# EndlessReform/fish-speech.rs

Measured on AMD Instinct MI355X. Metric: codec tokens/sec (frames/s; 1 frame = 1 slow + 8 codebook tokens = 2048 PCM samples), Fish-1.5 batch=1, higher is better.
Workload: dtype bf16

## Files before the change

fish-speech.rs_amd/csrc/lm_engine.hip:

```cpp
#include "lm_engine.h"

#include <algorithm>
#include <array>
#include <cmath>
#include <cstdlib>
#include <cstring>
#include <chrono>
#include <condition_variable>
#include <initializer_list>
#include <map>
#include <mutex>
#include <type_traits>
#include <vector>

#include <fcntl.h>
#include <sys/file.h>
#include <sys/stat.h>
#include <unistd.h>

#include "fs_common.h"
#include "fs_synth.h"
#include "lm_kernels.h"
#include "lm_persist.h"
#include "lm_persist_rows.h"
// ... 135 lines not shown
            throw Error("no HIP device visible: libfishrt has no CPU fallback (MI355X / gfx950 required)");
        FS_REQUIRE(device >= 0 && device < ndev, "device_id out of range");
        FS_HIP(hipSetDevice(device));
        hipDeviceProp_t prop;
        FS_HIP(hipGetDeviceProperties(&prop, device));
        if (std::string(prop.gcnArchName).rfind("gfx950", 0) != 0)
            throw Error(std::string("libfishrt kernels are built for gfx950 only; device reports ") + prop.gcnArchName);
        FS_HIP(hipStreamCreateWithFlags(&st_, hipStreamNonBlocking));
        d_.dim = a.dim; d_.inter = a.intermediate_size; d_.H = a.n_head; d_.Hk = a.n_local_heads; d_.Dh = a.head_dim;
        d_.n_rep = a.n_head / a.n_local_heads; d_.eps = a.norm_eps;
        legacy_ = !t.has_semantic_end;
        generic_ = !legacy_ && t.im_end_id + 1 != t.semantic_start_id;
        if (!legacy_) FS_REQUIRE(t.semantic_start_id >= 1 && t.semantic_start_id < (uint32_t)a.vocab_size, "semantic_start_id outside the vocabulary");
        n_audio_ = legacy_ ? 2 : (generic_ ? a.vocab_size - (int)t.semantic_start_id + 1 : a.vocab_size - (int)t.im_end_id);
        if (legacy_) FS_REQUIRE(t.pad_id < (uint32_t)a.vocab_size, "pad_id outside the vocabulary");
        plan_tensors();
        alloc_runtime();
        for (auto& e : ev_) FS_HIP(hipEventCreate(&e));
        for (auto& e : ev_batch_) FS_HIP(hipEventCreateWithFlags(&e, hipEventDisableTiming));
    }
    ~LM() override {
        (void)hipSetDevice(device_);
        (void)hipStreamSynchronize(st_);
        destroy_graphs();
        for (auto& e : ev_) if (e) (void)hipEventDestroy(e);
        for (auto& e : ev_batch_) if (e) (void)hipEventDestroy(e);
        if (h_pin_) (void)hipHostFree(h_pin_);
        for (auto& hb : hid_pool_) (void)hipFree(hb.first);
        for (const HidSlot& h : sess_hid_) if (h.rows) (void)hipFree(h.rows);
        for (auto* q : {&sess_flight_, &sess_queue_})
// ... 313 lines not shown
            use_persist_ = plock.owns_lock() && persist_ok_ && batch_rows_ == 0 &&
                           (cfg.temp == 0.f || fast_persist_samples(cfg.temp, cfg.top_k, a_.codebook_size));
            use_pslow_ = plock.owns_lock() && pslow_ok_;
        }
        if (hidden_out && !d_hidden_.p) d_hidden_.alloc(sizeof(float) * (size_t)out_cap_ * a_.dim);
        float* hid_dev = hidden_out ? d_hidden_.as<float>() : nullptr;
        FS_HIP(hipMemcpyAsync(d_hid_slot_.p, &hid_dev, sizeof(hid_dev), hipMemcpyHostToDevice, st_));
        RngState rng;
        upload_rng(seed, rng, d_rng_.as<RngState>(), st_);
        SeqState ss = {};
        ss.pos = n_cached; ss.prompt_L = L;
        FS_HIP(hipMemcpyAsync(state(0), &ss, sizeof(ss), hipMemcpyHostToDevice, st_));
        FS_HIP(hipMemcpyAsync(d_prompt_.p, prompt, sizeof(uint32_t) * C1 * L, hipMemcpyHostToDevice, st_));
        launch_reppen_reset(rp_, C, a_.codebook_size, st_);
        clear_fast();

        stats_ = {};
        FS_HIP(hipEventRecord(ev_[0], st_));
        prefill_tokens(0, L - 1, true);
        LmKernels<WT>::embed(d_, tok_emb_, cb_emb_, C, a_.codebook_size, d_cfg_.as<SampleCfg>(), d_prompt_.as<uint32_t>(), state(0),
                             x(0), st_);
        GenRun g;
        g.T0 = n_cached + L; g.n_iter = n_iter; g.cb = cb; g.cb_user = cb_user;
        g.time_k = (flags & FS_GEN_TIME_KERNELS) && use_persist_ && use_pslow_ && fold_slow_sampler();
        if constexpr (std::is_same<WT, bf16_t>::value) {
            if (getenv("FISHRT_B1_ROWS_FAST") && use_persist_ && use_pslow_ && fold_slow_sampler() && !legacy_) {
                ensure_rows(2);
                g.b1_rows_fast = true;
                const int big = 1 << 30;
                FS_HIP(hipMemcpyAsync(d_rcfg_.p, &cfg, sizeof(cfg), hipMemcpyHostToDevice, st_));
// ... 54 lines not shown

    struct GenRun {
        int T0 = 0;
        long long n_iter = 0;
        fs_frame_cb cb = nullptr;
        void* cb_user = nullptr;
        bool time_k = false, b1_rows_fast = false, multi_ok = false;
        std::vector<hipEvent_t> kev;
        long long it = 1;
        size_t delivered = 0;
        bool stop = false, ended = false;
    };
    void gen_frame(GenRun& g, long long it_) {
        set_bucket(g.T0 + (int)it_);
        if (g.b1_rows_fast) {
            launch_slow_persist(pslow_args(), st_);
            RowsFastArgs F = rows_fast_args(0, 1);
            F.slow_logits = d_logits_slow_.as<float>();
            F.cap = nullptr;
            launch_rows_fast(F, 1, persist_sampled_, st_);
            return;
        }
        if (g.time_k && it_ >= 1) {
            for (int i = 0; i < 3; ++i) { hipEvent_t e; FS_HIP(hipEventCreate(&e)); g.kev.push_back(e); }
            FS_HIP(hipEventRecord(g.kev[g.kev.size() - 3], st_));
            launch_slow_persist(pslow_args(), st_);
            FS_HIP(hipEventRecord(g.kev[g.kev.size() - 2], st_));
            launch_fast_persist(persist_args(), persist_sampled_, st_);
            FS_HIP(hipEventRecord(g.kev[g.kev.size() - 1], st_));
            return;
        }
// ... 1606 lines not shown
                if (FP8) d_sscl_.alloc(sizeof(float) * slow_persist_scale_floats(a_.n_layer));
                d_snorms_.alloc(sizeof(float) * (size_t)(2 * a_.n_layer + 1) * a_.dim);
                d_sedges_.alloc(slow_persist_edge_bytes());
                FS_HIP(hipMemset(d_sedges_.p, 0, d_sedges_.n));
                d_sctl_.alloc(320);
                FS_HIP(hipMemset(d_sctl_.p, 0, d_sctl_.n));
            }
            std::vector<const float*> np;
            for (int l = 0; l < a_.n_layer; ++l) { np.push_back(slow_[l].attn_norm); np.push_back(slow_[l].ffn_norm); }
            np.push_back(norm_w_);
            if (FP8) launch_slow_persist_pack_fp8(slow_.data(), a_.n_layer, slow_head_w(), slow_head_s(), n_audio_, np.data(), d_spack_.p, d_hpack_.p,
                                                  d_sscl_.as<float>(), d_snorms_.as<float>(), st_);
            else launch_slow_persist_pack(slow_.data(), a_.n_layer, slow_head_w(), n_audio_, np.data(), d_spack_.p, d_hpack_.p, d_snorms_.as<float>(), st_);
            FS_HIP(hipStreamSynchronize(st_));
            pslow_ok_ = true;
        }
    }
    SlowPersistArgs pslow_args() {
        SlowPersistArgs A = {};
        A.wpack = d_spack_.p; A.hpack = d_hpack_.p; A.norms = d_snorms_.as<float>();
        A.scales = d_sscl_.p ? d_sscl_.as<float>() : nullptr;
        A.hscales = d_sscl_.p ? d_sscl_.as<float>() + (size_t)a_.n_layer * PF_BLOCKS * 48 : nullptr;
        A.n_layer = a_.n_layer; A.n_head_rows = n_audio_;
        A.cos_t = d_cos_.as<float>(); A.sin_t = d_sin_.as<float>(); A.eps = d_.eps;
        A.x = x(0); A.logits = d_logits_slow_.as<float>(); A.state = state(0);
        A.kv_pool = kv_pool_.p; A.layer_half = (size_t)n_pages_ * page_elems_;
        A.page_table = d_page_table_.as<int>();
        A.n_sl = std::min(nc_launch_, nc_launch_ > 32 ? 16 : 8);
        if (const char* c = getenv("FISHRT_NSL_MAX")) A.n_sl = std::max(1, std::min(A.n_sl, atoi(c)));
        if (const char* c = getenv("FISHRT_NSL_MIN")) A.n_sl = std::min(16, std::max(A.n_sl, atoi(c)));
        while (A.n_sl & (A.n_sl - 1)) A.n_sl &= A.n_sl - 1;
        A.edges = d_sedges_.as<unsigned long long>();
        A.ctl = d_sctl_.as<uint32_t>();
        A.prof = getenv("FISHRT_PERSIST_PROF") ? reinterpret_cast<unsigned long long*>(d_sctl_.as<uint32_t>() + 16) : nullptr;
        A.peer_stamps = (A.prof && d_ctl_.p) ? reinterpret_cast<const unsigned long long*>(d_ctl_.as<uint32_t>() + 16) + 16 : nullptr;
        set_naps(A.naps, "FISHRT_NAPS_SLOW", kFp8 ? kNapsSlowFp8 : kNapsSlow);
        A.prof_wg = getenv("FISHRT_PERSIST_PROF_WG") ? atoi(getenv("FISHRT_PERSIST_PROF_WG")) : 0;
        A.l2_touch = getenv("FISHRT_SLOW_EARLY") ? atoi(getenv("FISHRT_SLOW_EARLY")) : (kFp8 ? 1 : 9);
        return A;
    }
    bool fold_slow_sampler() const { return use_persist_ && n_audio_ <= 2048; }
    FastPersistArgs persist_args() {
        FastPersistArgs A = {};
        A.wpack = d_pack_.p;
        A.scales = d_fscl_.p ? d_fscl_.as<float>() : nullptr;
        for (int l = 0; l < PF_LAYERS; ++l) { A.norms[2 * l] = fast_[l].attn_norm; A.norms[2 * l + 1] = fast_[l].ffn_norm; }
        A.norms[2 * PF_LAYERS] = fast_norm_w_;
        A.fast_emb = fast_emb_; A.tok_emb = tok_emb_; A.cb_emb = cb_emb_;
        A.qkv0_tbl = d_qkv0_.p ? d_qkv0_.as<float>() : nullptr;
        A.cos_t = d_cos_.as<float>(); A.sin_t = d_sin_.as<float>();
        A.eps = d_.eps;
        const bool fold = fold_slow_sampler();
        A.xf = fold ? x(0) : xf(0); A.x = x(0);
        A.slow_logits = fold ? d_logits_slow_.as<float>() : nullptr; A.n_slow = n_audio_; A.hid_slot = d_hid_slot_.as<float*>();
        A.cap = d_cap_.as<float>(); A.cap_frames = cap_frames_;
        A.state = state(0); A.cfg = d_cfg_.as<SampleCfg>(); A.rp = rp_; A.rng = d_rng_.as<RngState>();
        A.out_codes = d_out_.as<uint32_t>(); A.out_cap = out_cap_;
        A.edges = d_edges_.as<unsigned long long>();
        A.ctl = d_ctl_.as<uint32_t>();
        A.prof = getenv("FISHRT_PERSIST_PROF") ? reinterpret_cast<unsigned long long*>(d_ctl_.as<uint32_t>() + 16) : nullptr;
        A.peer_stamps = (A.prof && d_sctl_.p) ? reinterpret_cast<const unsigned long long*>(d_sctl_.as<uint32_t>() + 16) + 16 : nullptr;
        set_naps(A.naps, "FISHRT_NAPS_FAST", persist_sampled_ ? kNapsFastSampled : kNapsFast);
        return A;
    }


    void ensure_rows(int R) {
        if constexpr (std::is_same<WT, bf16_t>::value || kFp8) {
// ... 75 lines not shown
        A.slow_logits = d_rlogits_.as<float>() + (size_t)r0 * PR_LD; A.n_slow = n_audio_;
        A.cap = cap_frames_ ? d_rcap_.as<float>() + (size_t)r0 * cap_frames_ * 9 * 2048 : nullptr; A.cap_frames = cap_frames_;
        A.state = state(r0); A.cfg = d_rcfg_.as<SampleCfg>() + r0; A.budget = d_rbudget_.as<int>() + r0; A.rng = d_rrng_.as<RngState>() + r0;
        const RepPenState rp = rows_rp(r0);
        A.rp_mask = rp.mask; A.rp_ring = rp.ring; A.rp_meta = rp.ring_meta;
        A.out_codes = d_out_.as<uint32_t>() + (size_t)r0 * a_.num_codebooks * out_cap_; A.out_cap = out_cap_;
        A.edges = d_redges_f_.as<unsigned long long>();
        A.ctl = d_rctl_f_.as<uint32_t>();
        A.prof = getenv("FISHRT_PERSIST_PROF") ? reinterpret_cast<unsigned long long*>(d_rctl_f_.as<uint32_t>() + 16) : nullptr;
        set_naps(A.naps, "FISHRT_NAPS_ROWS_FAST", kNapsRowsFast);
        A.nap_draw = getenv("FISHRT_NAP_ROWS_DRAW") ? atoi(getenv("FISHRT_NAP_ROWS_DRAW")) : 16;
        return A;
    }
    FastPersistArgs persist_args(int i) {
        FastPersistArgs A = persist_args();
        A.xf = x(i); A.x = x(i);
        A.slow_logits = d_rlogits_.as<float>() + (size_t)i * PR_LD;
        A.cap = cap_frames_ ? d_rcap_.as<float>() + (size_t)i * cap_frames_ * 9 * 2048 : nullptr;
        A.state = state(i); A.cfg = d_rcfg_.as<SampleCfg>() + i; A.rp = rows_rp(i); A.rng = d_rrng_.as<RngState>() + i;
        A.out_codes = d_out_.as<uint32_t>() + (size_t)i * a_.num_codebooks * out_cap_;
        return A;
    }

    void enqueue_slow_layers(int b) {
        for (int l = 0; l < a_.n_layer; ++l) {
            const LayerW& w = slow_[l];
            KVView kv = slow_kv(l, b);
            LmKernels<WT>::qkv(d_, x(b), w, d_cos_.as<float>(), d_sin_.as<float>(), state(b), 0, 0, d_q_.as<float>(), kv, st_);
            LmKernels<WT>::attn_decode(d_, d_q_.as<float>(), kv, state(b), d_part_.as<float>(), n_chunks_, nc_launch_, st_);
            LmKernels<WT>::wo(d_, d_part_.as<float>(), n_chunks_, nc_launch_, state(b), nullptr, kv, 0, w, x(b), st_);
            LmKernels<WT>::ffn_up(d_, x(b), w, d_act_.as<float>(), st_);
// ... 102 lines not shown
            launch_fast_persist(persist_args(), persist_sampled_, st_);
        }
        FS_HIP(hipStreamEndCapture(st_, &g));
        FS_HIP(hipGraphInstantiate(&ge, g, nullptr, nullptr, 0));
        FS_HIP(hipGraphDestroy(g));
        multi_graphs_[key] = ge;
        return ge;
    }
    size_t page_elems_ = 0;
    DevBuf kv_pool_, fast_pool_, d_page_table_, d_zero_table_;
    std::vector<int> free_pages_, seq_len_, fast_len_;
    std::vector<std::vector<int>> seq_pages_;
    DevBuf d_x_, d_xf_, d_q_, d_part_, d_act_, d_logits_slow_, d_logits_fast_, d_state_, d_cfg_, d_rng_, d_prompt_, d_out_;
    DevBuf d_rp_mask_, d_rp_seen_, d_rp_ring_, d_rp_meta_;
    DevBuf d_pack_, d_edges_, d_ctl_, d_qkv0_;
    DevBuf d_fscl_, d_sscl_;
    DevBuf d_cap_;
    int cap_frames_ = 0;
    DevBuf d_hidden_, d_hid_slot_;
    bool persist_ok_ = false, use_persist_ = false, pslow_ok_ = false, use_pslow_ = false, persist_sampled_ = false;
    int batch_rows_ = 0, batch_row_ = 0;
    bool sess_active_ = false, sess_rows_ = false, sess_sampled_ = false;
    bool sess_slots_ = false;
    SampleCfg sess_cfg_ = {};
    DevBuf d_scfg_, d_srng_, d_srp_mask_, d_srp_seen_, d_srp_ring_, d_srp_meta_;
    int sess_R_ = 0, sess_adds_ = 0, sess_budget_tmp_ = 0;
    uint64_t sess_seed_ = 0;
    std::unique_lock<PersistLock> sess_plock_;
    std::vector<int> sess_left_, sess_pos_;
    std::vector<SeqState> sess_hs_;
// ... 72 lines not shown
```

fish-speech.rs_amd/csrc/lm_persist.h:

```cpp
#pragma once
#include <hip/hip_runtime.h>

#include <cstdint>

#include "lm_kernels.h"

namespace fs {

constexpr int PF_BLOCKS = 256;
constexpr int PF_THREADS = 512;
constexpr int PF_REPL = 8;
constexpr int PF_EDGE_CAP = 4096;
constexpr int PF_RING = 4;
constexpr int PF_LAYERS = 4;
constexpr int PF_REG_DW = PF_LAYERS * (5 + 4 + 32) + 4;
constexpr int PF_REG_CHUNKS = PF_REG_DW / 4;
constexpr int PF_ROW_CHUNKS = (PF_LAYERS * 9 + 4) / 4;
constexpr int PF_LDS_CHUNKS = PF_LAYERS * 4;
constexpr int PF_CHUNKS = PF_REG_CHUNKS + PF_LDS_CHUNKS;
constexpr int PF_SCL = 200;

struct FastPersistArgs {
    const void* wpack;
    const float* scales;
    const float* norms[2 * PF_LAYERS + 1];
    const void* fast_emb;
    const float* qkv0_tbl;
    const void* tok_emb;
    const void* cb_emb;
    const float* cos_t;
    const float* sin_t;
    float eps;
    const float* xf;
    const float* slow_logits;
    int n_slow;
    float* cap;
    int cap_frames;
    float* const* hid_slot;
    float* x;
    SeqState* state;
    const SampleCfg* cfg;
    RepPenState rp;
    RngState* rng;
    uint32_t* out_codes;
    int out_cap;
    unsigned long long* edges;
    unsigned long long* prof;
    const unsigned long long* peer_stamps;
    uint32_t* ctl;
    int naps[6];
};

constexpr int PS_EDGE_CAP = 16 * 16 * 66 + 64;
constexpr size_t PS_LAYER_IMAGE = 116736;
// ... 12 lines not shown
    const float* sin_t;
    float eps;
    float* x;
    float* logits;
    const SeqState* state;
    void* kv_pool;
    size_t layer_half;
    const int* page_table;
    int n_sl;
    unsigned long long* edges;
    unsigned long long* prof;
    const unsigned long long* peer_stamps;
    uint32_t* ctl;
    int naps[6];
    int prof_wg;
    int l2_touch;
};
size_t slow_persist_pack_bytes(int n_layer, bool fp8 = false);
size_t slow_persist_scale_floats(int n_layer);
void launch_slow_persist_pack_fp8(const LayerW* layers, int n_layer, const void* head_w, const float* head_s, int n_head_rows,
                                  const float* const* norm_ptrs, void* wpack, void* hpack, float* scales, float* norms_flat, hipStream_t st);
size_t slow_persist_edge_bytes();
void launch_slow_persist_pack(const LayerW* layers, int n_layer, const void* head_w, int n_head_rows, const float* const* norm_ptrs,
                              void* wpack, void* hpack, float* norms_flat, hipStream_t st);
void launch_slow_persist(const SlowPersistArgs& a, hipStream_t st);

bool fast_persist_supported(const ModelDims& d, int n_fast_layer, int n_cb, int cb_size);
size_t fast_persist_pack_bytes();
size_t fast_persist_edge_bytes();
void launch_fast_persist_pack(const LayerW* fast, const void* head_w, void* pack, hipStream_t st, bool fp8 = false, const float* head_s = nullptr,
// ... 10 lines not shown
```

fish-speech.rs_amd/csrc/lm_persist.hip:

```cpp
#include "lm_persist.h"

#include <hip/hip_runtime.h>

#include "fs_common.h"

namespace fs {

namespace {

#include "lm_persist_dev.h"
#include "lm_bsample_dev.h"

typedef __bf16 bf16x8_t __attribute__((ext_vector_type(8)));
typedef float f32x4_t __attribute__((ext_vector_type(4)));

constexpr int L_W2 = 0;
constexpr int L_KC = L_W2 + PF_LDS_CHUNKS * PF_THREADS * 16;
constexpr int L_VC = L_KC + PF_LAYERS * 8 * 64 * 4;
constexpr int L_QS = L_VC + PF_LAYERS * 8 * 64 * 4;
constexpr int L_XS = L_QS + 4096;
constexpr int PF_RED = 40;
constexpr int L_RED = L_XS + 4096;
constexpr int L_SC = L_RED + 2 * 8 * PF_RED * 4;
constexpr int L_AMAX = L_SC + 16 * 8 * 4;
// ... 223 lines not shown
            __syncthreads();
        }
        if (cap && tid == 0) cap[2047] = (float)idx;
        cur0 = audio_tok(cfg, max(idx, 0));
        if (cur0 == cfg.im_end_id) done_in = 1;
    }
    const bool eos = cur0 == cfg.im_end_id;
    if (eos && b != 0) return;

    bool dead = false;
    float x0 = 0.f, x1 = 0.f;
    unsigned long long tk[16] = {0, 0, 0, 0, 0, 0, 0, 0, 0, 0, 0, 0, 0, 0, 0, 0}, t_last = A.prof ? wall_clock64() : 0;
    const unsigned long long t_timers = t_last;
#define PF_TICK(k) do { if (A.prof) { const unsigned long long n_ = wall_clock64(); tk[k] += n_ - t_last; t_last = n_; } } while (0)
    if (!eos) {
        const u32x4* wp = reinterpret_cast<const u32x4*>(A.wpack) + (size_t)b * PF_CHUNKS * PF_THREADS + tid;
        uint32_t wr[4 * PF_ROW_CHUNKS];
        u32x4 w13v[PF_LAYERS][8];
#pragma unroll
        for (int c = 0; c < PF_ROW_CHUNKS; ++c) {
            const u32x4 t4 = wp[(size_t)c * PF_THREADS];
            wr[4 * c] = t4.x; wr[4 * c + 1] = t4.y; wr[4 * c + 2] = t4.z; wr[4 * c + 3] = t4.w;
        }
#pragma unroll
        for (int c = PF_ROW_CHUNKS; c < PF_REG_CHUNKS; ++c) w13v[(c - PF_ROW_CHUNKS) / 8][(c - PF_ROW_CHUNKS) % 8] = wp[(size_t)c * PF_THREADS];
#pragma unroll
        for (int c = 0; c < PF_LDS_CHUNKS; ++c) w2s[c * PF_THREADS + tid] = wp[(size_t)(PF_REG_CHUNKS + c) * PF_THREADS];
        float2 nwr[2 * PF_LAYERS + 1];
        if (!SAMPLED) {
#pragma unroll
// ... 11 lines not shown
            const float2 xin = *reinterpret_cast<const float2*>(A.xf + 2 * tid);
            x0 = xin.x; x1 = xin.y;
        }
        asm volatile("s_waitcnt vmcnt(0)" ::: "memory");
#pragma unroll
        for (int d = 0; d < 4 * PF_ROW_CHUNKS; ++d) asm volatile("" : "+v"(wr[d]));
#pragma unroll
        for (int l = 0; l < PF_LAYERS; ++l)
#pragma unroll
            for (int u2 = 0; u2 < 8; ++u2) asm volatile("" : "+v"(w13v[l][u2]));

        PF_TICK(0);
        unsigned e = 0;
        const unsigned tag0 = epoch * 256u;
        int par = 0;
        float2 tq = make_float2(0.f, 0.f), tk2 = tq, tv2 = tq;
        float xres_tbl = 0.f;
#pragma unroll 1
        for (int cb = 0; cb < 8; ++cb) {
            const int T = cb + 1;
#pragma unroll
            for (int l = 0; l < PF_LAYERS; ++l) {
                const uint32_t* wl = wr + 9 * l;
                const bool from_tbl = l == 0 && cb > 0 && A.qkv0_tbl != nullptr;
                if (!from_tbl) {
                    tid = pf_opaque(tid_k); lane = tid & 63; wave = tid >> 6;
                    const float2 nw = norm_w(2 * l, tid);
                    if (l > 0) {
                        u32x4 v;
                        pf_nap_before_sweep(A.naps[0]);
                        pf_sweep1(my_edges + (size_t)(e & 3) * PF_REPL * PF_EDGE_CAP, tid, tag0 + e + 1, v, dead, A.ctl);
                        x0 = __uint_as_float(v.x); x1 = __uint_as_float(v.z);
                        ++e;
                        PF_TICK(9);
                    }
                    if ((unsigned)(2 * tid - 4 * b) < 4u) *reinterpret_cast<float2*>(xr + 2 * tid - 4 * b) = make_float2(x0, x1);
                    const float xn0 = x0 * nw.x, xn1 = x1 * nw.y;
                    float a8[8];
#pragma unroll
// ... 313 lines not shown
                        tk2 = *reinterpret_cast<const float2*>(row + 1024 + g2 * 64 + 2 * j2);
                        tv2 = *reinterpret_cast<const float2*>(row + 1152 + g2 * 64 + 2 * j2);
                        const uint32_t hw = reinterpret_cast<const uint16_t*>(A.fast_emb)[(size_t)code * 1024 + 4 * b + min(tid & 15, 3)];
                        xres_tbl = __uint_as_float(hw << 16);
                    } else {
                        const uint32_t ew = reinterpret_cast<const uint32_t*>(A.fast_emb)[(size_t)code * 512 + tid];
                        x0 = bf_lo(ew); x1 = bf_hi(ew);
                    }
                }
            }
        }
    } else if (tid < 8) {
        s_misc[4 + tid] = 0;
        A.state->cur[tid + 1] = 0;
    }
    if (b != 0) return;
    __syncthreads();
    uint32_t* cur = s_prev;
    if (tid == 0) cur[0] = cur0;
    else if (tid <= 8) cur[tid] = s_misc[3 + tid];
    __syncthreads();
    if (tid == 0) {
        SeqState* st = A.state;
        const int frame = st->frame;
        if (done_in == 1) st->done = 2;
        if (A.slow_logits) st->cur[0] = cur0;
        if (frame == 0 || cur0 != cfg.im_end_id) {
            const int o = st->n_out;
            if (o < A.out_cap)
                for (int cc = 0; cc < 8; ++cc) A.out_codes[(size_t)cc * A.out_cap + o] = cur[cc + 1];
            st->n_out = o + 1;
        }
        for (int i = 0; i <= 8; ++i) st->prev[i] = cur[i];
        st->have_prev = 1;
        st->pos += 1;
        st->frame = frame + 1;
        if (SAMPLED || (cfg.legacy && A.slow_logits)) A.rng->consumed = consumed0 + (unsigned long long)n_draws;
        A.ctl[0] = epoch + 1;
    }
    {
        const uint32_t sem = cur[0];
        const float m = (sem >= cfg.sem_lo && sem <= cfg.sem_hi) ? 1.f : 0.f;
        const uint32_t* te = reinterpret_cast<const uint32_t*>(A.tok_emb);
        const uint32_t* ce = reinterpret_cast<const uint32_t*>(A.cb_emb);
        const uint32_t w0 = te[(size_t)sem * 512 + tid];
        float e0 = 0.f + bf_lo(w0), e1 = 0.f + bf_hi(w0);
#pragma unroll
        for (int c = 0; c < 8; ++c) {
            const uint32_t wv = ce[((size_t)c * 1024 + cur[c + 1]) * 512 + tid];
            e0 += bf_lo(wv) * m;
            e1 += bf_hi(wv) * m;
        }
        *reinterpret_cast<float2*>(A.x + 2 * tid) = make_float2(e0, e1);
    }
    PF_TICK(7);
    if (A.prof && tid == 0) {
        for (int k = 0; k < 16; ++k) A.prof[k] += tk[k];
        const unsigned long long t_end = wall_clock64(), peer_end = A.peer_stamps ? A.peer_stamps[0] : 0;
        if (peer_end && t_entry > peer_end && t_entry - peer_end < 20000) { A.prof[17] += t_entry - peer_end; A.prof[20] += 1; }
        A.prof[18] += t_timers - t_entry;
        A.prof[19] += t_end - t_last;
        A.prof[16] = t_end;
    }
#undef PF_TICK
}

__global__ __launch_bounds__(64) void k_pf_reduce_selftest(const float* __restrict__ in, float* __restrict__ out) {
    const int lane = threadIdx.x;
    float v32[32], v16[16], v8[8], v4[4];
// ... 63 lines not shown
```

fish-speech.rs_amd/csrc/lm_persist_slow.hip:

```cpp
#include "lm_persist.h"

#include <hip/hip_runtime.h>

#include <type_traits>
#include <vector>

#include "fs_common.h"

namespace fs {

namespace {

#include "lm_persist_dev.h"
#include "lm_persist_rows_dev.h"

constexpr int PS_DROR8 = 0x128;

constexpr size_t IM_QKV4 = 0, IM_QKV1 = 8192, IM_WO = 10240, IM_W13 = 18432, IM_W2 = 83968;
static_assert(IM_W2 + 4 * 8192 == PS_LAYER_IMAGE, "image layout");
constexpr size_t I8_QKV4 = 0, I8_QKV1 = 4096, I8_WO = 6144, I8_W13 = 10240, I8_W2 = 43008;
static_assert(I8_W2 + 2 * 8192 == PS_LAYER_IMAGE_FP8, "fp8 image layout");
constexpr int PS_SC = 48, SC_QKV = 0, SC_WO = 8, SC_W13 = 12, SC_W2 = 44;

typedef float f32x2_t __attribute__((ext_vector_type(2)));
// ... 165 lines not shown
    const unsigned epoch = A.ctl[0];
    const unsigned tag0 = epoch * 256u;
    const int n_sl = A.n_sl;
    const bool att = b < 16 * n_sl;
    const int ah = att ? b / n_sl : 0, as = att ? b % n_sl : 0, ag = ah >> 3;
    const int chunk_t = (pos + n_sl - 1) / n_sl;
    const int t0 = min(pos, as * chunk_t), t1 = min(pos, (as + 1) * chunk_t);
    const bool last_slice = att && as == n_sl - 1;
    const int n_tok = t1 - t0;
    const int n_tiles = att ? max((n_tok + 127) / 128, last_slice ? 1 : 0) : 0;
    if (att) {
        const int p0 = t0 >> 6;
        for (int i = tid; i < 160; i += PF_THREADS) s_pages[i] = (n_tok > 0 && p0 + i <= ((t1 - 1) >> 6)) ? A.page_table[p0 + i] : 0;
    }
    const int page_new = A.page_table[pos >> 6];
    float2 x2 = *reinterpret_cast<const float2*>(A.x + 2 * tid);
    float x0 = x2.x, x1 = x2.y;
    float rope_c = A.cos_t[(size_t)rpos * 32 + (tid & 31)], rope_s = A.sin_t[(size_t)rpos * 32 + (tid & 31)];
    __syncthreads();
    asm volatile("" : "+v"(rope_c), "+v"(rope_s));

    constexpr size_t LIMG = FP8 ? PS_LAYER_IMAGE_FP8 : PS_LAYER_IMAGE;
    const unsigned char* wimg = reinterpret_cast<const unsigned char*>(A.wpack) + (size_t)b * LIMG;
    const size_t layer_img = (size_t)PF_BLOCKS * LIMG;
    u32x4 wq4 = u32x4{0, 0, 0, 0}, wo4 = u32x4{0, 0, 0, 0}, w13[8], w2r[4];
    u32x2 wq4f = u32x2{0, 0}, wo4f = u32x2{0, 0};
    u32x4 w13f[4], w2f[2];
    uint32_t wq1;
    if constexpr (FP8) {
        wq4f = reinterpret_cast<const u32x2*>(wimg + I8_QKV4)[tid];
        wq1 = reinterpret_cast<const uint32_t*>(wimg + I8_QKV1)[tid];
    } else {
        wq4 = reinterpret_cast<const u32x4*>(wimg + IM_QKV4)[tid];
        wq1 = reinterpret_cast<const uint32_t*>(wimg + IM_QKV1)[tid];
    }
// ... 65 lines not shown
        const unsigned char* wl = wimg + (size_t)l * layer_img;
        {
            tid = pf_opaque(tid_k); lane = tid & 63; wave = tid >> 6;
            const float2 nw = *reinterpret_cast<const float2*>(A.norms + (size_t)(2 * l) * 1024 + 2 * tid);
            if (l > 0) {
                u32x4 v;
                pf_nap_before_sweep(A.naps[0]);
                pf_sweep1(my_edges + (size_t)(e & 3) * ering, tid, tag0 + e + 1, v, dead, A.ctl);
                x0 = __uint_as_float(v.x); x1 = __uint_as_float(v.z);
                ++e;
                PS_TICK(9);
            }
            const bool kv_late = (early_mode & 8) != 0;
            if (att && n_tok > 0 && !kv_late) load_kv_tile0(l);
            *reinterpret_cast<float2*>(xs + 2 * tid) = make_float2(x0, x1);
            const float xn0 = x0 * nw.x, xn1 = x1 * nw.y;
            float a8[8] = {0.f, 0.f, 0.f, 0.f, 0.f, 0.f, 0.f, 0.f};
            float rsc = 1.f;
            if constexpr (FP8) {
                if (tid < 64) rsc = scl[(size_t)l * scl_layer + SC_QKV + min(tid & 15, 4)];
                pf_dot2x2_fp8(wq4f.x, xn0, xn1, a8[0], a8[1]); pf_dot2x2_fp8(wq4f.y, xn0, xn1, a8[2], a8[3]);
                pf_dot2x2_fp8(wq1, xn0, xn1, a8[4], a8[6]);
                a8[6] = 0.f;
            } else {
                a8[0] = pf_dot2(wq4.x, xn0, xn1, 0.f); a8[1] = pf_dot2(wq4.y, xn0, xn1, 0.f);
                a8[2] = pf_dot2(wq4.z, xn0, xn1, 0.f); a8[3] = pf_dot2(wq4.w, xn0, xn1, 0.f);
                a8[4] = pf_dot2(wq1, xn0, xn1, 0.f);
            }
            a8[5] = fmaf(x1, x1, fmaf(x0, x0, 0.f));
            const float r8 = pf_reduce<8>(a8, lane);
            if ((lane & 7) == 0) red[(par * 8 + wave) * PS_RED + (lane >> 3)] = r8;
            __syncthreads();
            if (wave == 0) {
                const int r = min(lane & 15, 5), k = lane >> 4;
                const float* rp = red + (par * 8 + k) * PS_RED;
                float t = pf_sum_rows(rp[r] + rp[4 * PS_RED + r]);
                const float tot = pf_sum_rows(rp[5] + rp[4 * PS_RED + 5]);
                if constexpr (FP8) t *= rsc;
                if ((lane & 15) < 5) {
                    const float val = t * pf_rms_inv(tot, A.eps);
                    pub(e, k, 5 * b + r, tag0 + e + 1, val);
                    pub(e, k + 4, 5 * b + r, tag0 + e + 1, val);
                }
            }
            if (att && n_tok > 0 && kv_late) load_kv_tile0(l);
            if (early13) request_w13(wl);
            if (early2) request_w2(wl);
            par ^= 1;
            PS_TICK(1);
        }
        if constexpr (FP8) wo4f = reinterpret_cast<const u32x2*>(wl + I8_WO)[tid];
        else wo4 = reinterpret_cast<const u32x4*>(wl + IM_WO)[tid];
        if (att) {
            tid = pf_opaque(tid_k); lane = tid & 63; wave = tid >> 6;
            const u64* eb = my_edges + (size_t)(e & 3) * ering;
            if (tid < 96) {
                const int unit = tid < 32 ? 32 * ah + tid : (tid < 64 ? 512 + 32 * ag + (tid - 32) : 576 + 32 * ag + (tid - 64));
                u32x4 v;
                pf_nap_before_sweep(A.naps[1]);
                pf_sweep1(eb, unit, tag0 + e + 1, v, dead, A.ctl);
                const float a0 = __uint_as_float(v.x), a1 = __uint_as_float(v.z);
                const int j = tid & 31;
                const float c = rope_c, s = rope_s;
                if (tid < 32) {
                    *reinterpret_cast<float2*>(qs + 2 * j) = make_float2((a0 * c - a1 * s) * 0.125f, (a0 * s + a1 * c) * 0.125f);
                } else if (tid < 64) {
                    const uint32_t k0 = f32_to_bf16_rne(a0 * c - a1 * s), k1 = f32_to_bf16_rne(a0 * s + a1 * c);
                    *reinterpret_cast<float2*>(knew + 2 * j) = make_float2(bf_lo(k0), bf_lo(k1));
                    if (last_slice && (ah & 7) == 0)
                        reinterpret_cast<uint32_t*>(reinterpret_cast<uint16_t*>(A.kv_pool) + (size_t)l * 2 * A.layer_half +
                                                    ((size_t)(page_new * 2 + ag) * KV_PAGE + (pos & 63)) * 64)[j] = k0 | (k1 << 16);
                } else {
                    const uint32_t v0 = f32_to_bf16_rne(a0), v1 = f32_to_bf16_rne(a1);
                    *reinterpret_cast<float2*>(vnew + 2 * j) = make_float2(bf_lo(v0), bf_lo(v1));
                    if (last_slice && (ah & 7) == 0)
                        reinterpret_cast<uint32_t*>(reinterpret_cast<uint16_t*>(A.kv_pool) + (size_t)l * 2 * A.layer_half + A.layer_half +
                                                    ((size_t)(page_new * 2 + ag) * KV_PAGE + (pos & 63)) * 64)[j] = v0 | (v1 << 16);
                }
            }
            ++e;
            __syncthreads();
            PS_TICK(10);
            float run_m = -1e30f, run_l = 0.f, ro[8] = {0.f, 0.f, 0.f, 0.f, 0.f, 0.f, 0.f, 0.f};
            const int du = tid & 7;
            float qv[8];
            {
                const float4 q0 = *reinterpret_cast<const float4*>(qs + du * 8), q1 = *reinterpret_cast<const float4*>(qs + du * 8 + 4);
                qv[0] = q0.x; qv[1] = q0.y; qv[2] = q0.z; qv[3] = q0.w; qv[4] = q1.x; qv[5] = q1.y; qv[6] = q1.z; qv[7] = q1.w;
            }
            for (int tile = 0; tile < n_tiles; ++tile) {
                if (tile > 0) load_kv_tile(l, tile);
                float sc[3];
                bool valid[3];
#pragma unroll
                for (int u = 0; u < 2; ++u) {
// ... 63 lines not shown
                float M = wmax[0];
#pragma unroll
                for (int w = 1; w < 8; ++w) M = fmaxf(M, wmax[w]);
                float val = 0.f;
                if (tid == 64) val = M;
                else {
#pragma unroll
                    for (int w = 0; w < 8; ++w) val = fmaf(part[w * 72 + (tid < 64 ? tid : 64)], __expf(wmax[w] - M), val);
                }
                const int base = (ah * n_sl + as) * 66;
#pragma unroll
                for (int rr = 0; rr < PF_REPL; ++rr) pub(e, rr, base + tid, tag0 + e + 1, val);
            }
            __syncthreads();
            PS_TICK(2);
        } else {
            ++e;
        }
        {
            tid = pf_opaque(tid_k); lane = tid & 63; wave = tid >> 6;
            const int h = tid >> 5, j = tid & 31;
            const u64* eb = my_edges + (size_t)(e & 3) * ering;
            float rsc = 1.f;
            if constexpr (FP8) { if (tid < 64) rsc = scl[(size_t)l * scl_layer + SC_WO + min(tid & 15, 3)]; }
            float mn = -1e30f, L = 0.f, at0 = 0.f, at1 = 0.f;
            float sm[16], sl_[16], so0[16], so1[16];
            pf_nap_before_sweep(A.naps[2]);
            if (n_sl > 4) {
                const unsigned off_o = (unsigned)((h * n_sl * 66 + 2 * j) * 8), off_ml = (unsigned)((h * n_sl * 66 + 64) * 8);
#pragma unroll
                for (int rd = 0; rd < 2; ++rd) {
// ... 250 lines not shown
                    pub(e, k, 4 * b + r, tag0 + e + 1, xres + t);
                    pub(e, k + 4, 4 * b + r, tag0 + e + 1, xres + t);
                }
            }
            par ^= 1;
            PS_TICK(5);
        }
    }
    {
        tid = pf_opaque(tid_k); lane = tid & 63; wave = tid >> 6;
        const float2 nw = *reinterpret_cast<const float2*>(A.norms + (size_t)(2 * A.n_layer) * 1024 + 2 * tid);
        const u32x4* hp = reinterpret_cast<const u32x4*>(reinterpret_cast<const unsigned char*>(A.hpack) + (size_t)b * (FP8 ? PS_HEAD_IMAGE_FP8 : PS_HEAD_IMAGE));
        const u32x4 h0 = hp[tid], h1 = FP8 ? u32x4{0, 0, 0, 0} : hp[PF_THREADS + tid];
        float rsc = 1.f;
        if constexpr (FP8) { if (tid < 64) rsc = A.hscales[8 * b + min(tid & 15, 7)]; }
        u32x4 v;
        pf_nap_before_sweep(A.naps[5]);
        pf_sweep1(my_edges + (size_t)(e & 3) * ering, tid, tag0 + e + 1, v, dead, A.ctl);
        ++e;
        PS_TICK(14);
        x0 = __uint_as_float(v.x); x1 = __uint_as_float(v.z);
        if (b == 0) *reinterpret_cast<float2*>(A.x + 2 * tid) = make_float2(x0, x1);
        const float xn0 = x0 * nw.x, xn1 = x1 * nw.y;
        float a8[8] = {0.f, 0.f, 0.f, 0.f, 0.f, 0.f, 0.f, 0.f};
        if constexpr (FP8) {
            pf_dot2x2_fp8(h0.x, xn0, xn1, a8[0], a8[1]); pf_dot2x2_fp8(h0.y, xn0, xn1, a8[2], a8[3]);
            pf_dot2x2_fp8(h0.z, xn0, xn1, a8[4], a8[5]); pf_dot2x2_fp8(h0.w, xn0, xn1, a8[6], a8[7]);
        } else {
            a8[0] = pf_dot2(h0.x, xn0, xn1, 0.f); a8[1] = pf_dot2(h0.y, xn0, xn1, 0.f); a8[2] = pf_dot2(h0.z, xn0, xn1, 0.f); a8[3] = pf_dot2(h0.w, xn0, xn1, 0.f);
            a8[4] = pf_dot2(h1.x, xn0, xn1, 0.f); a8[5] = pf_dot2(h1.y, xn0, xn1, 0.f); a8[6] = pf_dot2(h1.z, xn0, xn1, 0.f); a8[7] = pf_dot2(h1.w, xn0, xn1, 0.f);
        }
        const float ssw = pf_wave_sum(fmaf(x1, x1, fmaf(x0, x0, 0.f)));
        const float r8 = pf_reduce<8>(a8, lane);
        if ((lane & 7) == 0) red[(par * 8 + wave) * PS_RED + (lane >> 3)] = r8;
        if (lane == 0) red[(par * 8 + wave) * PS_RED + 8] = ssw;
        __syncthreads();
        if (wave == 0) {
            const int r = min(lane & 15, 7), k = lane >> 4;
            const float* rp = red + (par * 8 + k) * PS_RED;
            float t = pf_sum_rows(rp[r] + rp[4 * PS_RED + r]);
            const float tot = pf_sum_rows(rp[8] + rp[4 * PS_RED + 8]);
            if constexpr (FP8) t *= rsc;
            if (lane < 8 && 8 * b + r < A.n_head_rows) A.logits[8 * b + r] = t * pf_rms_inv(tot, A.eps);
        }
        PS_TICK(6);
    }
    if (b == 0 && tid == 0) A.ctl[0] = epoch + 1;
    if (A.prof && b == A.prof_wg && tid == 0) {
        for (int k = 0; k < 16; ++k) A.prof[k] += tk[k];
        const unsigned long long t_end = wall_clock64(), peer_end = A.peer_stamps ? A.peer_stamps[0] : 0;
        if (peer_end && t_entry > peer_end && t_entry - peer_end < 20000) { A.prof[17] += t_entry - peer_end; A.prof[20] += 1; }
        A.prof[18] += t_timers - t_entry;
        A.prof[19] += t_end - t_last;
        A.prof[16] = t_end;
    }
#undef PS_TICK
}

// ... 46 lines not shown
```

Baseline: 1872.

## Hand off layer-0 QKV projections across slow/fast persistent kernel boundaries

At the end of the slow persistent kernel, the fast transformer's layer-0 QKV projection is computed from the final hidden state and handed to the fast kernel. At the end of the fast kernel, the next slow step's layer-0 QKV is computed from the new embedding and tagged with an epoch. Each receiving kernel skips its first layer's QKV matvec and the edge-exchange sweep that goes with it. This takes one cross-workgroup sync round off each kernel's critical path, at the cost of extra weight loads and reductions in the tail of the previous kernel. It also adds more complex tag and epoch handling, and for FP8 builds only the slow-to-fast handoff is enabled.

```diff
diff --git a/fish-speech.rs_amd/csrc/lm_engine.hip b/fish-speech.rs_amd/csrc/lm_engine.hip
--- a/fish-speech.rs_amd/csrc/lm_engine.hip
+++ b/fish-speech.rs_amd/csrc/lm_engine.hip
@@ -173,6 +173,8 @@
         if (!legacy_) FS_REQUIRE(t.semantic_start_id >= 1 && t.semantic_start_id < (uint32_t)a.vocab_size, "semantic_start_id outside the vocabulary");
         n_audio_ = legacy_ ? 2 : (generic_ ? a.vocab_size - (int)t.semantic_start_id + 1 : a.vocab_size - (int)t.im_end_id);
         if (legacy_) FS_REQUIRE(t.pad_id < (uint32_t)a.vocab_size, "pad_id outside the vocabulary");
+        if (const char* e = getenv("FISHRT_BOUNDARY_QKV")) boundary_qkv_ = atoi(e) & 3;
+        if (kFp8) boundary_qkv_ &= 1;
         plan_tensors();
         alloc_runtime();
         for (auto& e : ev_) FS_HIP(hipEventCreate(&e));
@@ -516,6 +518,7 @@
         FS_HIP(hipMemcpyAsync(d_prompt_.p, prompt, sizeof(uint32_t) * C1 * L, hipMemcpyHostToDevice, st_));
         launch_reppen_reset(rp_, C, a_.codebook_size, st_);
         clear_fast();
+        boundary_reset();
 
         stats_ = {};
         FS_HIP(hipEventRecord(ev_[0], st_));
@@ -600,7 +603,9 @@
     void gen_frame(GenRun& g, long long it_) {
         set_bucket(g.T0 + (int)it_);
         if (g.b1_rows_fast) {
-            launch_slow_persist(pslow_args(), st_);
+            SlowPersistArgs S = pslow_args();
+            S.fast_qkv0 = nullptr; S.qkv0_in = nullptr;
+            launch_slow_persist(S, st_);
             RowsFastArgs F = rows_fast_args(0, 1);
             F.slow_logits = d_logits_slow_.as<float>();
             F.cap = nullptr;
@@ -2237,8 +2242,20 @@
             else launch_slow_persist_pack(slow_.data(), a_.n_layer, slow_head_w(), n_audio_, np.data(), d_spack_.p, d_hpack_.p, d_snorms_.as<float>(), st_);
             FS_HIP(hipStreamSynchronize(st_));
             pslow_ok_ = true;
-        }
-    }
+            if ((boundary_qkv_ & 1) && !d_fqkv0_.p) {
+                d_fqkv0_.alloc(sizeof(float) * 1280);
+                FS_HIP(hipMemset(d_fqkv0_.p, 0, d_fqkv0_.n));
+            }
+            if ((boundary_qkv_ & 2) && !d_sqkv0_.p) {
+                d_sqkv0_.alloc(sizeof(float) * 1280 + 64);
+                FS_HIP(hipMemset(d_sqkv0_.p, 0xFF, d_sqkv0_.n));
+            }
+        }
+    }
+    float* boundary_fast_qkv0() { return (use_persist_ && use_pslow_ && fold_slow_sampler()) ? d_fqkv0_.as<float>() : nullptr; }
+    float* boundary_slow_qkv0() { return (use_persist_ && use_pslow_ && fold_slow_sampler()) ? d_sqkv0_.as<float>() : nullptr; }
+    uint32_t* boundary_slow_tag() { return reinterpret_cast<uint32_t*>(d_sqkv0_.as<float>() + 1280); }
+    void boundary_reset() { if (d_sqkv0_.p) FS_HIP(hipMemsetAsync(boundary_slow_tag(), 0xFF, sizeof(uint32_t), st_)); }
     SlowPersistArgs pslow_args() {
         SlowPersistArgs A = {};
         A.wpack = d_spack_.p; A.hpack = d_hpack_.p; A.norms = d_snorms_.as<float>();
@@ -2260,6 +2277,11 @@
         set_naps(A.naps, "FISHRT_NAPS_SLOW", kFp8 ? kNapsSlowFp8 : kNapsSlow);
         A.prof_wg = getenv("FISHRT_PERSIST_PROF_WG") ? atoi(getenv("FISHRT_PERSIST_PROF_WG")) : 0;
         A.l2_touch = getenv("FISHRT_SLOW_EARLY") ? atoi(getenv("FISHRT_SLOW_EARLY")) : (kFp8 ? 1 : 9);
+        if (float* q0 = boundary_fast_qkv0()) {
+            A.fast_wpack = d_pack_.p; A.fast_norm0 = fast_[0].attn_norm; A.fast_qkv0 = q0;
+            A.fast_scales = d_fscl_.p ? d_fscl_.as<float>() : nullptr;
+        }
+        if (float* q0 = boundary_slow_qkv0()) { A.qkv0_in = q0; A.qkv0_tag = boundary_slow_tag(); }
         return A;
     }
     bool fold_slow_sampler() const { return use_persist_ && n_audio_ <= 2048; }
@@ -2275,6 +2297,11 @@
         A.eps = d_.eps;
         const bool fold = fold_slow_sampler();
         A.xf = fold ? x(0) : xf(0); A.x = x(0);
+        A.qkv0_in = boundary_fast_qkv0();
+        if (float* q0 = boundary_slow_qkv0()) {
+            A.slow_wpack = d_spack_.p; A.slow_norm0 = d_snorms_.as<float>(); A.slow_qkv0 = q0;
+            A.slow_ctl = d_sctl_.as<uint32_t>(); A.slow_qkv0_tag = boundary_slow_tag();
+        }
         A.slow_logits = fold ? d_logits_slow_.as<float>() : nullptr; A.n_slow = n_audio_; A.hid_slot = d_hid_slot_.as<float*>();
         A.cap = d_cap_.as<float>(); A.cap_frames = cap_frames_;
         A.state = state(0); A.cfg = d_cfg_.as<SampleCfg>(); A.rp = rp_; A.rng = d_rng_.as<RngState>();
@@ -2380,7 +2407,7 @@
     }
     FastPersistArgs persist_args(int i) {
         FastPersistArgs A = persist_args();
-        A.xf = x(i); A.x = x(i);
+        A.xf = x(i); A.x = x(i); A.qkv0_in = nullptr; A.slow_qkv0 = nullptr;
         A.slow_logits = d_rlogits_.as<float>() + (size_t)i * PR_LD;
         A.cap = cap_frames_ ? d_rcap_.as<float>() + (size_t)i * cap_frames_ * 9 * 2048 : nullptr;
         A.state = state(i); A.cfg = d_rcfg_.as<SampleCfg>() + i; A.rp = rows_rp(i); A.rng = d_rrng_.as<RngState>() + i;
@@ -2513,6 +2540,9 @@
     DevBuf d_x_, d_xf_, d_q_, d_part_, d_act_, d_logits_slow_, d_logits_fast_, d_state_, d_cfg_, d_rng_, d_prompt_, d_out_;
     DevBuf d_rp_mask_, d_rp_seen_, d_rp_ring_, d_rp_meta_;
     DevBuf d_pack_, d_edges_, d_ctl_, d_qkv0_;
+    DevBuf d_fqkv0_;
+    DevBuf d_sqkv0_;
+    int boundary_qkv_ = 3;
     DevBuf d_fscl_, d_sscl_;
     DevBuf d_cap_;
     int cap_frames_ = 0;
diff --git a/fish-speech.rs_amd/csrc/lm_persist.h b/fish-speech.rs_amd/csrc/lm_persist.h
--- a/fish-speech.rs_amd/csrc/lm_persist.h
+++ b/fish-speech.rs_amd/csrc/lm_persist.h
@@ -32,12 +32,18 @@
     const float* sin_t;
     float eps;
     const float* xf;
+    const float* qkv0_in;
     const float* slow_logits;
     int n_slow;
     float* cap;
     int cap_frames;
     float* const* hid_slot;
     float* x;
+    const void* slow_wpack;
+    const float* slow_norm0;
+    float* slow_qkv0;
+    const uint32_t* slow_ctl;
+    uint32_t* slow_qkv0_tag;
     SeqState* state;
     const SampleCfg* cfg;
     RepPenState rp;
@@ -80,6 +86,12 @@
     uint32_t* ctl;
     int naps[6];
     int prof_wg;
+    const void* fast_wpack;
+    const float* fast_norm0;
+    const float* fast_scales;
+    float* fast_qkv0;
+    const float* qkv0_in;
+    const uint32_t* qkv0_tag;
     int l2_touch;
 };
 size_t slow_persist_pack_bytes(int n_layer, bool fp8 = false);
diff --git a/fish-speech.rs_amd/csrc/lm_persist.hip b/fish-speech.rs_amd/csrc/lm_persist.hip
--- a/fish-speech.rs_amd/csrc/lm_persist.hip
+++ b/fish-speech.rs_amd/csrc/lm_persist.hip
@@ -261,6 +261,16 @@
     const unsigned long long t_timers = t_last;
 #define PF_TICK(k) do { if (A.prof) { const unsigned long long n_ = wall_clock64(); tk[k] += n_ - t_last; t_last = n_; } } while (0)
     if (!eos) {
+        float2 tq = make_float2(0.f, 0.f), tk2 = tq, tv2 = tq;
+        float xres_tbl = 0.f;
+        const bool qkv0_handed = A.qkv0_in != nullptr;
+        if (qkv0_handed) {
+            const int h2 = tid >> 5, g2 = h2 >> 3, j2 = tid & 31;
+            tq = *reinterpret_cast<const float2*>(A.qkv0_in + 2 * tid);
+            tk2 = *reinterpret_cast<const float2*>(A.qkv0_in + 1024 + g2 * 64 + 2 * j2);
+            tv2 = *reinterpret_cast<const float2*>(A.qkv0_in + 1152 + g2 * 64 + 2 * j2);
+            xres_tbl = A.xf[4 * b + min(tid & 15, 3)];
+        }
         const u32x4* wp = reinterpret_cast<const u32x4*>(A.wpack) + (size_t)b * PF_CHUNKS * PF_THREADS + tid;
         uint32_t wr[4 * PF_ROW_CHUNKS];
         u32x4 w13v[PF_LAYERS][8];
@@ -302,15 +312,13 @@
         unsigned e = 0;
         const unsigned tag0 = epoch * 256u;
         int par = 0;
-        float2 tq = make_float2(0.f, 0.f), tk2 = tq, tv2 = tq;
-        float xres_tbl = 0.f;
 #pragma unroll 1
         for (int cb = 0; cb < 8; ++cb) {
             const int T = cb + 1;
 #pragma unroll
             for (int l = 0; l < PF_LAYERS; ++l) {
                 const uint32_t* wl = wr + 9 * l;
-                const bool from_tbl = l == 0 && cb > 0 && A.qkv0_tbl != nullptr;
+                const bool from_tbl = l == 0 && (cb > 0 ? A.qkv0_tbl != nullptr : qkv0_handed);
                 if (!from_tbl) {
                     tid = pf_opaque(tid_k); lane = tid & 63; wave = tid >> 6;
                     const float2 nw = norm_w(2 * l, tid);
@@ -654,13 +662,24 @@
         s_misc[4 + tid] = 0;
         A.state->cur[tid + 1] = 0;
     }
-    if (b != 0) return;
+    const bool hand = A.slow_qkv0 != nullptr && !eos;
+    if (b != 0 && !hand) return;
+    u32x4 sq4 = u32x4{0, 0, 0, 0};
+    uint32_t sq1 = 0u;
+    float2 snw = make_float2(0.f, 0.f);
+    if (hand) {
+        const unsigned char* im = reinterpret_cast<const unsigned char*>(A.slow_wpack) + (size_t)b * PS_LAYER_IMAGE;
+        sq4 = reinterpret_cast<const u32x4*>(im)[tid_k];
+        sq1 = reinterpret_cast<const uint32_t*>(im + 8192)[tid_k];
+        snw = *reinterpret_cast<const float2*>(A.slow_norm0 + 2 * tid_k);
+    }
+    tid = pf_opaque(tid_k); lane = tid & 63; wave = tid >> 6;
     __syncthreads();
     uint32_t* cur = s_prev;
     if (tid == 0) cur[0] = cur0;
     else if (tid <= 8) cur[tid] = s_misc[3 + tid];
     __syncthreads();
-    if (tid == 0) {
+    if (b == 0 && tid == 0) {
         SeqState* st = A.state;
         const int frame = st->frame;
         if (done_in == 1) st->done = 2;
@@ -677,6 +696,7 @@
         st->frame = frame + 1;
         if (SAMPLED || (cfg.legacy && A.slow_logits)) A.rng->consumed = consumed0 + (unsigned long long)n_draws;
         A.ctl[0] = epoch + 1;
+        if (hand) *A.slow_qkv0_tag = A.slow_ctl[0];
     }
     {
         const uint32_t sem = cur[0];
@@ -691,8 +711,27 @@
             e0 += bf_lo(wv) * m;
             e1 += bf_hi(wv) * m;
         }
-        *reinterpret_cast<float2*>(A.x + 2 * tid) = make_float2(e0, e1);
-    }
+        if (b == 0) *reinterpret_cast<float2*>(A.x + 2 * tid) = make_float2(e0, e1);
+        if (hand) {
+            const float xn0 = e0 * snw.x, xn1 = e1 * snw.y;
+            float a8[8] = {0.f, 0.f, 0.f, 0.f, 0.f, 0.f, 0.f, 0.f};
+            a8[0] = pf_dot2(sq4.x, xn0, xn1, 0.f); a8[1] = pf_dot2(sq4.y, xn0, xn1, 0.f);
+            a8[2] = pf_dot2(sq4.z, xn0, xn1, 0.f); a8[3] = pf_dot2(sq4.w, xn0, xn1, 0.f);
+            a8[4] = pf_dot2(sq1, xn0, xn1, 0.f);
+            a8[5] = fmaf(e1, e1, fmaf(e0, e0, 0.f));
+            const float r8 = pf_reduce<8>(a8, lane);
+            if ((lane & 7) == 0) red[wave * PF_RED + (lane >> 3)] = r8;
+            __syncthreads();
+            if (wave == 0) {
+                const int r = min(lane & 15, 5), k = lane >> 4;
+                const float* rp = red + k * PF_RED;
+                const float t = pf_sum_rows(rp[r] + rp[4 * PF_RED + r]);
+                const float tot = pf_sum_rows(rp[5] + rp[4 * PF_RED + 5]);
+                if (lane < 5) A.slow_qkv0[5 * b + r] = t * pf_rms_inv(tot, A.eps);
+            }
+        }
+    }
+    if (b != 0) return;
     PF_TICK(7);
     if (A.prof && tid == 0) {
         for (int k = 0; k < 16; ++k) A.prof[k] += tk[k];
diff --git a/fish-speech.rs_amd/csrc/lm_persist_slow.hip b/fish-speech.rs_amd/csrc/lm_persist_slow.hip
--- a/fish-speech.rs_amd/csrc/lm_persist_slow.hip
+++ b/fish-speech.rs_amd/csrc/lm_persist_slow.hip
@@ -203,11 +203,18 @@
         for (int i = tid; i < 160; i += PF_THREADS) s_pages[i] = (n_tok > 0 && p0 + i <= ((t1 - 1) >> 6)) ? A.page_table[p0 + i] : 0;
     }
     const int page_new = A.page_table[pos >> 6];
+    const bool hand_in = A.qkv0_in != nullptr && A.qkv0_tag[0] == epoch;
+    float2 hqkv = make_float2(0.f, 0.f);
+    {
+        const int unit = !att || tid >= 96 ? 0 : (tid < 32 ? 32 * ah + tid : (tid < 64 ? 512 + 32 * ag + (tid - 32) : 576 + 32 * ag + (tid - 64)));
+        hqkv = *reinterpret_cast<const float2*>((hand_in ? A.qkv0_in : A.x) + (hand_in ? 2 * unit : 0));
+    }
     float2 x2 = *reinterpret_cast<const float2*>(A.x + 2 * tid);
     float x0 = x2.x, x1 = x2.y;
     float rope_c = A.cos_t[(size_t)rpos * 32 + (tid & 31)], rope_s = A.sin_t[(size_t)rpos * 32 + (tid & 31)];
     __syncthreads();
     asm volatile("" : "+v"(rope_c), "+v"(rope_s));
+    asm volatile("" : "+v"(hqkv.x), "+v"(hqkv.y));
 
     constexpr size_t LIMG = FP8 ? PS_LAYER_IMAGE_FP8 : PS_LAYER_IMAGE;
     const unsigned char* wimg = reinterpret_cast<const unsigned char*>(A.wpack) + (size_t)b * LIMG;
@@ -303,6 +310,7 @@
             const bool kv_late = (early_mode & 8) != 0;
             if (att && n_tok > 0 && !kv_late) load_kv_tile0(l);
             *reinterpret_cast<float2*>(xs + 2 * tid) = make_float2(x0, x1);
+            if (!(hand_in && l == 0)) {
             const float xn0 = x0 * nw.x, xn1 = x1 * nw.y;
             float a8[8] = {0.f, 0.f, 0.f, 0.f, 0.f, 0.f, 0.f, 0.f};
             float rsc = 1.f;
@@ -332,10 +340,11 @@
                     pub(e, k + 4, 5 * b + r, tag0 + e + 1, val);
                 }
             }
+            par ^= 1;
+            }
             if (att && n_tok > 0 && kv_late) load_kv_tile0(l);
             if (early13) request_w13(wl);
             if (early2) request_w2(wl);
-            par ^= 1;
             PS_TICK(1);
         }
         if constexpr (FP8) wo4f = reinterpret_cast<const u32x2*>(wl + I8_WO)[tid];
@@ -346,8 +355,11 @@
             if (tid < 96) {
                 const int unit = tid < 32 ? 32 * ah + tid : (tid < 64 ? 512 + 32 * ag + (tid - 32) : 576 + 32 * ag + (tid - 64));
                 u32x4 v;
-                pf_nap_before_sweep(A.naps[1]);
-                pf_sweep1(eb, unit, tag0 + e + 1, v, dead, A.ctl);
+                if (hand_in && l == 0) { v.x = __float_as_uint(hqkv.x); v.z = __float_as_uint(hqkv.y); }
+                else {
+                    pf_nap_before_sweep(A.naps[1]);
+                    pf_sweep1(eb, unit, tag0 + e + 1, v, dead, A.ctl);
+                }
                 const float a0 = __uint_as_float(v.x), a1 = __uint_as_float(v.z);
                 const int j = tid & 31;
                 const float c = rope_c, s = rope_s;
@@ -367,7 +379,7 @@
                                                     ((size_t)(page_new * 2 + ag) * KV_PAGE + (pos & 63)) * 64)[j] = v0 | (v1 << 16);
                 }
             }
-            ++e;
+            if (!(hand_in && l == 0)) ++e;
             __syncthreads();
             PS_TICK(10);
             float run_m = -1e30f, run_l = 0.f, ro[8] = {0.f, 0.f, 0.f, 0.f, 0.f, 0.f, 0.f, 0.f};
@@ -461,7 +473,7 @@
             }
             __syncthreads();
             PS_TICK(2);
-        } else {
+        } else if (!(hand_in && l == 0)) {
             ++e;
         }
         {
@@ -742,6 +754,18 @@
         const u32x4 h0 = hp[tid], h1 = FP8 ? u32x4{0, 0, 0, 0} : hp[PF_THREADS + tid];
         float rsc = 1.f;
         if constexpr (FP8) { if (tid < 64) rsc = A.hscales[8 * b + min(tid & 15, 7)]; }
+        const bool hand = A.fast_qkv0 != nullptr;
+        u32x4 f0 = u32x4{0, 0, 0, 0};
+        uint32_t f1 = 0u;
+        float2 fnw = make_float2(0.f, 0.f);
+        float fsc = 1.f;
+        if (hand) {
+            const u32x4* fp = reinterpret_cast<const u32x4*>(A.fast_wpack) + (size_t)b * PF_CHUNKS * PF_THREADS + tid;
+            f0 = fp[0];
+            f1 = reinterpret_cast<const uint32_t*>(fp + PF_THREADS)[0];
+            fnw = *reinterpret_cast<const float2*>(A.fast_norm0 + 2 * tid);
+            if (A.fast_scales && tid < 64) fsc = A.fast_scales[(size_t)b * PF_SCL + min(tid & 15, 4)];
+        }
         u32x4 v;
         pf_nap_before_sweep(A.naps[5]);
         pf_sweep1(my_edges + (size_t)(e & 3) * ering, tid, tag0 + e + 1, v, dead, A.ctl);
@@ -749,6 +773,17 @@
         PS_TICK(14);
         x0 = __uint_as_float(v.x); x1 = __uint_as_float(v.z);
         if (b == 0) *reinterpret_cast<float2*>(A.x + 2 * tid) = make_float2(x0, x1);
+        if (hand) {
+            const uint32_t fw[5] = {f0.x, f0.y, f0.z, f0.w, f1};
+            const float fx0 = x0 * fnw.x, fx1 = x1 * fnw.y;
+            float f8[8];
+#pragma unroll
+            for (int r = 0; r < 5; ++r) f8[r] = pf_dot2(fw[r], fx0, fx1, 0.f);
+            f8[5] = fmaf(x1, x1, fmaf(x0, x0, 0.f));
+            f8[6] = 0.f; f8[7] = 0.f;
+            const float q8 = pf_reduce<8>(f8, lane);
+            if ((lane & 7) == 0) red[(par * 8 + wave) * PS_RED + 16 + (lane >> 3)] = q8;
+        }
         const float xn0 = x0 * nw.x, xn1 = x1 * nw.y;
         float a8[8] = {0.f, 0.f, 0.f, 0.f, 0.f, 0.f, 0.f, 0.f};
         if constexpr (FP8) {
@@ -770,6 +805,14 @@
             const float tot = pf_sum_rows(rp[8] + rp[4 * PS_RED + 8]);
             if constexpr (FP8) t *= rsc;
             if (lane < 8 && 8 * b + r < A.n_head_rows) A.logits[8 * b + r] = t * pf_rms_inv(tot, A.eps);
+            if (hand) {
+                const int fr = min(lane & 15, 5);
+                const float* fq = rp + 16;
+                float ft = pf_sum_rows(fq[fr] + fq[4 * PS_RED + fr]);
+                const float ftot = pf_sum_rows(fq[5] + fq[4 * PS_RED + 5]);
+                if (A.fast_scales) ft *= fsc;
+                if (lane < 5) A.fast_qkv0[5 * b + fr] = ft * pf_rms_inv(ftot, A.eps);
+            }
         }
         PS_TICK(6);
     }
```

Result: slower. 1796 (-4.1%).
